# vbronetskyi/nclt-slam-project

Measured on AMD Instinct MI355X. Metric: relocalization frames/sec @640x480, 10k-landmark DB; Hamming-match HBM GB/s, higher is better.
Workload: dtype u8; 1 GPU; 640x480 BGR frames, 10000-record landmark DB (640000 descriptors, rows=fixed64), global relocalization tick per frame: ORB(500) + whole-DB mutual Hamming scan + top-25 PnP-RANSAC(200); frames resident in HBM, every frame's 96-byte result record written to pinned host memory by the tick's last kernel; distinct_frames=32, preroll_steps=20, streams=4, records=10000, descriptors=640000, parallelism=frames sharded across ranks, database replicated, no collective

## Files before the change

nclt-slam-project_amd/csrc/reloc_ctx.hip:

```cpp
#include <stdarg.h>
#include <stdlib.h>

#include "reloc_internal.h"

static thread_local char g_err[512] = "";

void reloc_set_error(const char *fmt, ...)
{
    va_list ap;
    va_start(ap, fmt);
    vsnprintf(g_err, sizeof(g_err), fmt, ap);
    va_end(ap);
}

RELOC_API const char *reloc_last_error(void) { return g_err; }

RELOC_API int reloc_device_count(void)
{
    int n = 0;
    if (hipGetDeviceCount(&n) != hipSuccess) return 0;
    return n;
}

template <typename T>
// ... 68 lines not shown
    int n = 0;
    if (hipGetDeviceCount(&n) != hipSuccess || n <= 0) {
        reloc_set_error("no HIP device available (libreloc_hip has no CPU fallback)");
        return nullptr;
    }
    if (device < 0 || device >= n || max_w < 64 || max_h < 64 || max_feat < 64) {
        reloc_set_error("reloc_create: bad arguments (device %d of %d, %dx%d, max_feat %d)", device, n,
                        max_w, max_h, max_feat);
        return nullptr;
    }
    if (hipSetDevice(device) != hipSuccess) {
        reloc_set_error("hipSetDevice(%d) failed", device);
        return nullptr;
    }
    reloc_ctx *c = new reloc_ctx();
    __atomic_add_fetch(&g_reloc_live_contexts, 1, __ATOMIC_RELAXED);
    c->device = device;
    c->max_w = max_w;
    c->max_h = max_h;
    c->max_feat = max_feat;
    hipDeviceProp_t prop;
    if (hipGetDeviceProperties(&prop, device) == hipSuccess) c->num_cu = prop.multiProcessorCount;
    if (hipStreamCreateWithFlags(&c->own_stream, hipStreamNonBlocking) != hipSuccess ||
        hipEventCreate(&c->t0) != hipSuccess || hipEventCreate(&c->t1) != hipSuccess) {
        reloc_set_error("stream/event creation failed");
        __atomic_sub_fetch(&g_reloc_live_contexts, 1, __ATOMIC_RELAXED);
        delete c;
        return nullptr;
    }
    c->stream = c->own_stream;
    c->prm.nfeatures = 500;
    c->prm.max_candidates = RELOC_MAX_CANDIDATES;
    c->prm.min_matches = RELOC_MIN_MATCHES;
    c->prm.min_inliers = RELOC_MIN_INLIERS;
    c->prm.ransac_iterations = RELOC_RANSAC_ITERATIONS;
    c->prm.global_max_candidates = RELOC_GLOBAL_MAX_CANDIDATES;
    c->prm.global_min_inliers = RELOC_GLOBAL_MIN_INLIERS;
    c->prm.accum_min_kpts = RELOC_ACCUM_MIN_KPTS;
    c->prm.candidate_radius_m = RELOC_CANDIDATE_RADIUS_M;
    c->prm.heading_tol_deg = RELOC_HEADING_TOL_DEG;
    c->prm.reproj_max_px = RELOC_REPROJ_MAX_PX;
    c->prm.ransac_reproj_px = RELOC_RANSAC_REPROJ_PX;
    c->prm.ransac_confidence = RELOC_RANSAC_CONFIDENCE;
    c->prm.consistency_m = RELOC_CONSISTENCY_M;
    c->prm.global_reproj_max_px = RELOC_GLOBAL_REPROJ_MAX_PX;
    c->prm.accum_min_dist_m = RELOC_ACCUM_MIN_DIST_M;
    c->prm.accum_depth_min_m = RELOC_ACCUM_DEPTH_MIN_M;
    c->prm.accum_depth_max_m = RELOC_ACCUM_DEPTH_MAX_M;
    c->prm.gray_coeff_bits = RELOC_GRAY_DEFAULT_BITS;
    c->prm.reserved0 = 0;
    if (const char *dev = getenv("RELOC_DEV"); dev && dev[0] == '1' && dev[1] == 0) {
        if (const char *e = getenv("RELOC_SCAN_GRID")) c->scan_grid = atoi(e);
        if (const char *e = getenv("RELOC_SCAN_GENS")) c->scan_gens = atoi(e);
        if (const char *e = getenv("RELOC_SCAN_NW")) c->scan_nw = atoi(e);
        if (const char *e = getenv("RELOC_SCAN_BATCH_GENS")) c->scan_batch_gens = atoi(e);
        if (const char *e = getenv("RELOC_SCAN_QUOTA_ROWS")) c->scan_quota_rows = atoi(e);
        if (const char *e = getenv("RELOC_LOCAL_TWO_STAGE")) c->local_two_stage = atoi(e) != 0;
    }
    if (ctx_alloc(c) != 0) {
        reloc_destroy(c);
        return nullptr;
    }
    return c;
}

RELOC_API void reloc_destroy(reloc_ctx *c)
{
    if (!c) return;
    (void)hipSetDevice(c->device);
    if (c->stream) (void)hipStreamSynchronize(c->stream);
    db_arrays_drop(c->db_share, c->db_desc, c->db_pts3d, c->db_kp2d, c->db_off, c->db_pose, c->db_xy_heading);
    void *ptrs[] = {c->pyr, c->blur, c->nms, c->rz_tab, c->pyr_tiles, c->hist, c->cand_cnt, c->cand_key, c->cand_resp,
                    c->kp_cnt, c->kp_key, c->kp_resp, c->f_xy, c->f_size, c->f_angle, c->f_resp, c->f_oct,
                    c->f_desc, c->f_count, c->frame_img, c->orb_const, c->dbg_cut, c->db_counts, c->topk_part, c->cand_ids, c->cand_n, c->m_qidx,
                    c->m_tidx, c->m_dist, c->m_n, c->p_obj, c->p_img, c->p_Rt, c->p_cnt, c->p_inl,
                    c->p_out, c->tick_res, c->accum_res, c->tick_flags, c->scan_ticket, c->clahe_plane, c->clahe_lut};
    for (void *p : ptrs)
        if (p) (void)hipFree(p);
    if (c->tick_res_host) (void)hipHostFree(c->tick_res_host);
    {
        DbArena &a = c->db_slot[1 - c->db_sel];
        db_arrays_drop(a.share, a.desc, a.pts3d, a.kp2d, a.off, a.pose, a.xy_heading);
        if (a.counts) (void)hipFree(a.counts);
        if (a.topk_part) (void)hipFree(a.topk_part);
    }
    for (int i = 0; i < 8; ++i)
        if (c->scratch[i]) (void)hipFree(c->scratch[i]);
    for (int k = 0; k < RELOC_PROF_N; ++k)
        if (c->prof[k].init)
            for (int i = 0; i < RELOC_PROF_RING; ++i) {
                (void)hipEventDestroy(c->prof[k].a[i]);
                (void)hipEventDestroy(c->prof[k].b[i]);
            }
    if (c->t0) (void)hipEventDestroy(c->t0);
    if (c->t1) (void)hipEventDestroy(c->t1);
    if (c->own_stream) (void)hipStreamDestroy(c->own_stream);
    __atomic_sub_fetch(&g_reloc_live_contexts, 1, __ATOMIC_RELAXED);
    delete c;
}

RELOC_API int reloc_get_params(reloc_ctx *c, reloc_params *out)
{
    ARG_CHECK_CTX(c, out, "reloc_get_params");
    *out = c->prm;
    return RELOC_OK;
}

// ... 184 lines not shown
```

nclt-slam-project_amd/csrc/reloc_internal.h:

```cpp
#pragma once
#include <hip/hip_runtime.h>
#include <stdint.h>
#include <stdio.h>
#include <string.h>

#include "../../include/reloc.h"
#include "../../include/reloc_spec.h"

#define RELOC_API extern "C" __attribute__((visibility("default")))
#define RELOC_PROF_RING 256

void reloc_set_error(const char *fmt, ...);

#define HIP_TRY(expr)                                                                      \
    do {                                                                                   \
        hipError_t e_ = (expr);                                                            \
        if (e_ != hipSuccess) {                                                            \
            reloc_set_error("%s failed: %s (%s:%d)", #expr, hipGetErrorString(e_), __FILE__, \
                            __LINE__);                                                     \
            return RELOC_E_HIP;                                                            \
        }                                                                                  \
    } while (0)

#define ARG_CHECK(cond, msg)                                 \
// ... 205 lines not shown
    int max_w = 0, max_h = 0, max_feat = 0;
    hipStream_t own_stream = nullptr;
    hipStream_t stream = nullptr;
    hipEvent_t t0 = nullptr, t1 = nullptr;
    int num_cu = 256;

    int prof_on = 0;
    struct ProfSlot { hipEvent_t a[RELOC_PROF_RING], b[RELOC_PROF_RING]; int n = 0; float total = 0.f; int launches = 0; bool init = false; } prof[RELOC_PROF_N];

    void *scratch[8] = {};
    int64_t scratch_bytes[8] = {};

    int orb_w = 0, orb_h = 0, orb_nfeat = 0;
    OrbLevel lev[NLEV];
    int64_t pyr_bytes = 0;
    uint8_t *pyr = nullptr;
    uint8_t *blur = nullptr;
    uint8_t *nms = nullptr;
    int32_t *rz_tab = nullptr;
    void *pyr_tiles = nullptr;
    int pyr_ntiles = 0, pyr_lds[NLEV + 1] = {}, pyr_lds_bytes = 0;
    int32_t *hist = nullptr;
    int32_t *cand_cnt = nullptr;
    uint32_t *cand_key = nullptr;
    float *cand_resp = nullptr;
    int32_t *kp_cnt = nullptr;
    uint32_t *kp_key = nullptr;
    float *kp_resp = nullptr;
    float *f_xy = nullptr, *f_size = nullptr, *f_angle = nullptr, *f_resp = nullptr;
    int32_t *f_oct = nullptr;
    uint8_t *f_desc = nullptr;
    int32_t *f_count = nullptr;
    uint8_t *frame_img = nullptr;
    void *orb_const = nullptr;
    char orb_tab_host[1024];
    int32_t *dbg_cut = nullptr;

    double K4[4] = {RELOC_FX, RELOC_FY, RELOC_CX, RELOC_CY};
    double b2c_t[3] = {0.35, 0.0, 0.18};
    double b2c_R[9] = {0, -1, 0, 0, 0, -1, 1, 0, 0};
    double dist[5] = {0, 0, 0, 0, 0};
    bool has_dist = false;

    double clahe_clip = 0.0;
    int clahe_tx = 0, clahe_ty = 0;
    uint8_t *clahe_plane = nullptr;
    uint8_t *clahe_lut = nullptr;

    reloc_params prm;
    int scan_grid = 0;
    int scan_gens = 0;
    int scan_batch_gens = 0;
    int scan_quota_rows = 1;
    int scan_nw = 0;
    uint32_t *scan_ticket = nullptr;

    DbArena db_slot[2];
    int db_sel = 0;
    bool db_shared = false;
    DbShare *db_share = nullptr;
    int64_t db_records = 0, db_rows = 0;
    int64_t db_cap_records = 0, db_cap_rows = 0;
    int db_max_rows = 0;
    uint8_t *db_desc = nullptr;
    float *db_pts3d = nullptr;
    float *db_kp2d = nullptr;
    int64_t *db_off = nullptr;
    double *db_pose = nullptr;
    double *db_xy_heading = nullptr;
    int32_t *db_counts = nullptr;
    unsigned long long *topk_part = nullptr;
    int topk_blocks = 0;
    AccumResult *accum_res = nullptr;
    int32_t *tick_flags = nullptr;

    int32_t *cand_ids = nullptr;
    int32_t *cand_n = nullptr;
    int32_t *m_qidx = nullptr, *m_tidx = nullptr, *m_dist = nullptr, *m_n = nullptr;
    float *p_obj = nullptr, *p_img = nullptr;
    double *p_Rt = nullptr;
    int32_t *p_cnt = nullptr;
    int32_t *p_inl = nullptr;
    PnpOut *p_out = nullptr;
    int exclusive_hint = -1;
    bool orb_latency_shape = true;
    bool latency_shapes = false;
    bool local_two_stage = false;
    TickResult *tick_res = nullptr;
    TickResult *tick_res_host = nullptr;
    bool tick_failed = false;
    int32_t tick_seq = 0;
    TickResult *tick_res_ext = nullptr;
};

int reloc_scratch(reloc_ctx *ctx, int slot, int64_t bytes, void **out);
void reloc_prof_begin(reloc_ctx *ctx, int which);
void reloc_prof_end(reloc_ctx *ctx, int which);

void db_arrays_drop(DbShare *&share, uint8_t *&desc, float *&pts3d, float *&kp2d, int64_t *&off, double *&pose, double *&xyh);
extern int g_reloc_live_contexts;
static inline bool ctx_alone(const reloc_ctx *c)
{
    return c->exclusive_hint > 0 || (c->exclusive_hint < 0 && __atomic_load_n(&g_reloc_live_contexts, __ATOMIC_RELAXED) == 1);
}

int launch_db_scan(reloc_ctx *ctx, const uint8_t *db_desc, const int64_t *db_off, int64_t n_rec,
                   const int32_t *rec_ids, const int32_t *n_ids_dev, int n_ids_max, const uint8_t *cur,
// ... 17 lines not shown
```

nclt-slam-project_amd/csrc/reloc_match.hip:

```cpp
#include <stdlib.h>
#include <new>
#include <type_traits>
#include <utility>

#include "reloc_internal.h"

typedef uint32_t u32;

__device__ __forceinline__ u32 bcnt_acc(u32 x, u32 acc)
{
    u32 r;
    asm("v_bcnt_u32_b32 %0, %1, %2" : "=v"(r) : "v"(x), "v"(acc));
    return r;
}
__device__ __forceinline__ u32 min_u16(u32 a, u32 b)
{
    u32 r;
    asm("v_min_u16 %0, %1, %2" : "=v"(r) : "v"(a), "v"(b));
    return r;
}
template <u32 IDX>
__device__ __forceinline__ u32 key_fma(u32 d, u32 c128)
{
    u32 r;
// ... 275 lines not shown
                for (; tc < tend; tc += 16)
                    scan_chunk<NJ, 16, true>(rec, n, tc, min(16, tend - tc), q, (u32)(cb * CB), rowkey, colbest, ncb == 1, lane);
            }
        }
        __syncthreads();
        u32 base = 0;
        for (int rb = 0; rb < n; rb += 64 * NW) {
            const int row = rb + tid;
            bool mutual = false;
            u32 key = 0;
            if (row < n && C > 0) {
                key = rowkey[row];
                const u32 col = key & 0xFFFFu;
                mutual = (colbest[col] & 0xFFFFu) == (u32)row;
            }
            const unsigned long long bal = __ballot(mutual);
            if (lane == 0) wsum[wave] = (u32)__popcll(bal);
            __syncthreads();
            u32 before = base;
            for (int w = 0; w < wave; ++w) before += wsum[w];
            u32 total = 0;
            for (int w = 0; w < NW; ++w) total += wsum[w];
            if (EMIT && mutual) {
                const u32 pos = before + (u32)__popcll(bal & ((1ull << lane) - 1ull));
                const int64_t o = (int64_t)it * emit_stride + pos;
                m_qidx[o] = row;
                m_tidx[o] = (int32_t)(key & 0xFFFFu);
                m_dist[o] = (int32_t)(key >> 16);
                if (mask.g_obj) {
                    const float *p3 = mask.g_pts3d + 3 * (row0 + row), *p2 = mask.g_xy + 2 * (size_t)(key & 0xFFFFu);
                    float *po = mask.g_obj + 3 * o, *pi = mask.g_img + 2 * o;
                    po[0] = p3[0]; po[1] = p3[1]; po[2] = p3[2];
                    pi[0] = p2[0]; pi[1] = p2[1];
                }
            }
            base += total;
            __syncthreads();
        }
        if (tid == 0) {
            if (counts) counts[EMIT ? it : r] = (int32_t)base;
            if (EMIT && m_n) m_n[it] = (int32_t)base;
        }
        advance();
    }
    if (ticket && tid == 0) {
        const int words = pool_frames * 8;
        if (atomicAdd(&ticket_pool[words * TICKET_STRIDE], 1u) == gridDim.x - 1) {
            for (int x = 0; x <= words; ++x)
                __hip_atomic_store(&ticket_pool[x * TICKET_STRIDE], 0u, __ATOMIC_RELAXED, __HIP_MEMORY_SCOPE_AGENT);
        }
    }
}

template <int NJ, int NW>
__device__ __forceinline__ void db_count_body(
    u32 *lds, int C, const uint4 *__restrict__ db, const int64_t *__restrict__ off, const int32_t *__restrict__ rec_ids,
    const int32_t *__restrict__ n_ids_p, int n_ids_max, const uint4 *__restrict__ cur, int max_rows,
    int32_t *__restrict__ counts, const ScanMask &mask, u32 *ticket, int quota, int n_bounded, int col_words,
    u32 *ticket_pool = nullptr, int pool_frames = 1, int block = -1, int n_blocks = -1)
{
    if (!ticket_pool) ticket_pool = ticket;
    if (block < 0) { block = blockIdx.x; n_blocks = gridDim.x; }
    constexpr int CB = 64 * NJ;
    const int tid = threadIdx.x, lane = tid & 63;
    const int wave = __builtin_amdgcn_readfirstlane(tid >> 6);
    const int n_ids = n_ids_p ? min(*n_ids_p, n_ids_max) : n_ids_max;
    const int ncb = max((C + CB - 1) / CB, 1);
    const bool dbl = 2 * ncb * CB <= col_words;
    u32 *colbuf = lds;
    u32 *rowkey = colbuf + col_words;
    u32 *wsum = rowkey + max_rows;

    u32 q[NJ][8];
    auto load_q = [&](int colbase) {
#pragma unroll
        for (int j = 0; j < NJ; ++j) {
            const int col = min(colbase + j * 64 + lane, max(C - 1, 0));
            const uint4 a = cur[2 * col], b = cur[2 * col + 1];
            q[j][0] = a.x; q[j][1] = a.y; q[j][2] = a.z; q[j][3] = a.w;
            q[j][4] = b.x; q[j][5] = b.y; q[j][6] = b.z; q[j][7] = b.w;
        }
    };
    const bool bound = (NW % ncb) == 0;
    const int my_cb = bound ? wave % ncb : 0;
    const int chunk0 = bound ? wave / ncb : wave, chunk_step = bound ? NW / ncb : NW;
    const bool stand_down = mask.skip_if && *mask.skip_if != 0;
    if (bound && !stand_down) load_q(my_cb * CB);
    double hc = 1.0, hs = 0.0, cos_tol = 0.0;
    if (mask.xyh) {
        cur_heading_q(mask.q, hc, hs);
        cos_tol = mask.cos_tol;
        hc = uniform_f64(hc); hs = uniform_f64(hs); cos_tol = uniform_f64(cos_tol);
    }
    constexpr int TICKET_STRIDE = 32;
    int shard = 0, dry = 0;
    if (ticket) {
        u32 x;
        asm volatile("s_getreg_b32 %0, hwreg(HW_REG_XCC_ID, 0, 4)" : "=s"(x));
        shard = (int)(x & 7u);
    }
    auto draw = [&]() -> u32 { return atomicAdd(&ticket[shard * TICKET_STRIDE], 1u); };
    auto settle = [&](u32 t) -> int {
        for (;;) {
            const long long rec_i = (long long)n_blocks + (long long)shard + 8ll * (long long)t;
            if (rec_i < n_ids) return (int)rec_i;
            if (++dry >= 8) return n_ids;
            shard = (shard + 1) & 7;
            t = draw();
        }
    };
    int it = stand_down ? n_ids : block;
    const bool by_rows = n_bounded >= 0;
    int left = (quota > 0 && (!by_rows || block < n_bounded)) ? quota : 0x7fffffff;
    for (int i = tid; i < ncb * CB; i += 64 * NW) colbuf[i] = 0xFFFFFFFFu;
    if (tid == 0) wsum[0] = wsum[1] = 0;
    __syncthreads();
    int p = 0;
    while (it < n_ids) {
        u32 *colbest = colbuf + (dbl ? p * ncb * CB : 0);
        const int r = rec_ids ? rec_ids[it] : it;
        const bool scored = !(mask.xyh && !heading_ok(mask.xyh + 4 * (int64_t)r, hc, hs, cos_tol));
        const int64_t row0 = off[r];
        const int n = scored ? (int)(off[r + 1] - row0) : 0;
        const uint4 *rec = db + 2 * row0;
        left -= by_rows ? max(n, 1) : 1;
        u32 next_ticket = 0;
        if (ticket && tid == 0 && left > 0) next_ticket = draw();
        if (n > 0 && C > 0) {
            if (ncb > 1) {
                for (int i = tid; i < n; i += 64 * NW) rowkey[i] = 0xFFFFFFFFu;
                __syncthreads();
            }
            for (int cb = bound ? my_cb : 0; cb < (bound ? my_cb + 1 : ncb); ++cb) {
                if (!bound) load_q(cb * CB);
                const int per = n / chunk_step, extra = n % chunk_step;
                int tc = chunk0 * per + min(chunk0, extra);
                const int tend = tc + per + (chunk0 < extra ? 1 : 0);
#pragma nounroll
                for (; tc < tend; tc += 16)
                    scan_chunk<NJ, 16, true>(rec, n, tc, min(16, tend - tc), q, (u32)(cb * CB), rowkey, colbest, ncb == 1, lane);
            }
        }
        if (dbl) {
            u32 *other = colbuf + (p ^ 1) * ncb * CB;
            for (int i = tid; i < ncb * CB; i += 64 * NW) other[i] = 0xFFFFFFFFu;
        }
        __syncthreads();
        if (C > 0) {
            for (int rb = 0; rb < n; rb += 64 * NW) {
                const int row = rb + tid;
                bool mutual = false;
                if (row < n) {
                    const u32 col = rowkey[row] & 0xFFFFu;
                    mutual = (colbest[col] & 0xFFFFu) == (u32)row;
                }
                const u32 c = (u32)__popcll(__ballot(mutual));
                if (lane == 0 && c) atomicAdd(&wsum[p], c);
            }
        }
        if (tid == 0) wsum[8] = ticket ? (left > 0 ? (u32)settle(next_ticket) : (u32)n_ids) : (u32)(it + n_blocks);
        __syncthreads();
        if (tid == 0) {
            counts[r] = (int32_t)wsum[p];
            wsum[p] = 0;
        }
        it = __builtin_amdgcn_readfirstlane((int)wsum[8]);
        if (dbl) p ^= 1;
        else {
            for (int i = tid; i < ncb * CB; i += 64 * NW) colbuf[i] = 0xFFFFFFFFu;
            __syncthreads();
        }
    }
    if (ticket && tid == 0) {
        const int words = pool_frames * 8;
        if (atomicAdd(&ticket_pool[words * TICKET_STRIDE], 1u) == gridDim.x - 1) {
            for (int x = 0; x <= words; ++x)
                __hip_atomic_store(&ticket_pool[x * TICKET_STRIDE], 0u, __ATOMIC_RELAXED, __HIP_MEMORY_SCOPE_AGENT);
        }
    }
}

template <int NJ, bool EMIT, int NW>
__global__ __launch_bounds__(64 * NW, NW >= 4 ? 16 / NW : 4) RELOC_SCAN_VGPR_ATTR void k_db_scan(
    const uint4 *__restrict__ db, const int64_t *__restrict__ off, const int32_t *__restrict__ rec_ids,
    const int32_t *__restrict__ n_ids_p, int n_ids_max, const uint4 *__restrict__ cur,
    const int32_t *__restrict__ n_cur_p, int n_cur_max, int max_rows, int32_t *__restrict__ counts,
    int32_t *__restrict__ m_qidx, int32_t *__restrict__ m_tidx, int32_t *__restrict__ m_dist,
    int32_t *__restrict__ m_n, int emit_stride, ScanMask mask, u32 *ticket, int quota, int n_bounded, int col_words)
{
    extern __shared__ u32 lds[];
    if constexpr (EMIT) RELOC_SMALL_KERNEL_PRIO();
    const int C = n_cur_p ? min(*n_cur_p, n_cur_max) : n_cur_max;
    if constexpr (EMIT)
        db_scan_body<NJ, true, NW>(lds, C, db, off, rec_ids, n_ids_p, n_ids_max, cur, max_rows, counts, m_qidx, m_tidx, m_dist, m_n,
                                   emit_stride, mask, ticket, quota);
    else
        db_count_body<NJ, NW>(lds, C, db, off, rec_ids, n_ids_p, n_ids_max, cur, max_rows, counts, mask, ticket, quota, n_bounded, col_words);
}

struct EmitFrame {
    const int32_t *rec_ids, *n_ids_p; const uint4 *cur; const int32_t *n_cur_p;
    int32_t *m_qidx, *m_tidx, *m_dist, *m_n; const float *g_xy; float *g_obj, *g_img;
};
struct EmitBatch { EmitFrame f[RELOC_BATCH_MAX]; };

__global__ __launch_bounds__(256, 4) RELOC_SCAN_VGPR_ATTR void k_db_emit_batch(const uint4 *__restrict__ db, const int64_t *__restrict__ off, int n_ids_max,
                                                          int n_cur_max, int max_rows, int emit_stride, const float *__restrict__ g_pts3d,
                                                          EmitBatch bt)
{
    extern __shared__ u32 lds[];
    RELOC_SMALL_KERNEL_PRIO();
    const EmitFrame &F = bt.f[blockIdx.y];
    ScanMask mask;
    mask.xyh = nullptr;
    mask.q[0] = mask.q[1] = mask.q[2] = 0; mask.q[3] = 1;
    mask.g_pts3d = g_pts3d; mask.g_xy = F.g_xy; mask.g_obj = F.g_obj; mask.g_img = F.g_img;
    const int C = F.n_cur_p ? min(*F.n_cur_p, n_cur_max) : n_cur_max;
    db_scan_body<8, true, 4>(lds, C, db, off, F.rec_ids, F.n_ids_p, n_ids_max, F.cur, max_rows, nullptr, F.m_qidx, F.m_tidx, F.m_dist, F.m_n,
                             emit_stride, mask, nullptr, 0);
}

int launch_db_emit_batch(reloc_ctx *const *ctxs, int n)
{
    reloc_ctx *c0 = ctxs[0];
    if (n < 1 || n > RELOC_BATCH_MAX) { reloc_set_error("emit batch: 1..%d frames", RELOC_BATCH_MAX); return RELOC_E_ARG; }
    if (c0->max_feat > 65535 || c0->db_max_rows > MAX_REC_ROWS) { reloc_set_error("emit batch: capacity"); return RELOC_E_CAPACITY; }
    EmitBatch bt;
    for (int f = 0; f < RELOC_BATCH_MAX; ++f) {
        reloc_ctx *c = ctxs[f < n ? f : 0];
        EmitFrame &F = bt.f[f];
        F.rec_ids = c->cand_ids; F.n_ids_p = c->cand_n; F.cur = (const uint4 *)c->f_desc; F.n_cur_p = c->f_count;
        F.m_qidx = c->m_qidx; F.m_tidx = c->m_tidx; F.m_dist = c->m_dist; F.m_n = c->m_n; F.g_xy = c->f_xy; F.g_obj = c->p_obj; F.g_img = c->p_img;
    }
    const int max_rows = c0->db_max_rows < 1 ? 1 : c0->db_max_rows;
    const int ncb = (c0->max_feat + 511) / 512;
    const size_t lds = (size_t)(ncb * 512 + max_rows + 16) * 4;
    if (lds > 160 * 1024) { reloc_set_error("emit batch: LDS demand %zu bytes", lds); return RELOC_E_CAPACITY; }
    hipLaunchKernelGGL(k_db_emit_batch, dim3(MAX_CAND, n), dim3(256), lds, c0->stream, (const uint4 *)c0->db_desc, c0->db_off, MAX_CAND,
                       c0->max_feat, max_rows, MAX_REC_ROWS, c0->db_pts3d, bt);
    HIP_TRY(hipGetLastError());
    return RELOC_OK;
}

constexpr int SCAN_BATCH_MAX = 8;
struct ScanBatch {
    int n;
    const uint4 *cur[SCAN_BATCH_MAX];
    const int32_t *n_cur[SCAN_BATCH_MAX];
    int32_t *counts[SCAN_BATCH_MAX];
    const int32_t *skip_if[SCAN_BATCH_MAX];
    double q[SCAN_BATCH_MAX][4];
    const double *xyh;
    double cos_tol;
};

__global__ __launch_bounds__(256, 4) RELOC_SCAN_VGPR_ATTR void k_db_scan_batch(const uint4 *__restrict__ db, const int64_t *__restrict__ off, int n_ids,
                                                          int n_cur_max, int max_rows, ScanBatch bt, u32 *ticket_pool, int quota, int n_bounded, int col_words)
{
    extern __shared__ u32 lds[];
    const int f = blockIdx.x % bt.n;
    ScanMask mask;
    mask.xyh = bt.xyh;
    for (int k = 0; k < 4; ++k) mask.q[k] = bt.q[f][k];
    mask.cos_tol = bt.cos_tol;
    mask.skip_if = bt.skip_if[f];
    const int C = bt.n_cur[f] ? min(*bt.n_cur[f], n_cur_max) : n_cur_max;
    db_count_body<8, 4>(lds, C, db, off, nullptr, nullptr, n_ids, bt.cur[f], max_rows, bt.counts[f], mask, ticket_pool + f * 8 * 32, quota,
                        n_bounded, col_words, ticket_pool, bt.n, (int)(blockIdx.x / bt.n), (int)((gridDim.x + bt.n - 1 - f) / bt.n));
}

__device__ __forceinline__ u32 max_u16(u32 a, u32 b)
{
    u32 r;
    asm("v_max_u16 %0, %1, %2" : "=v"(r) : "v"(a), "v"(b));
    return r;
}

__global__ __launch_bounds__(256, 4) void k_db_ratio(const uint4 *__restrict__ db, const int64_t *__restrict__ off, int n_rec,
                                                     const uint4 *__restrict__ cur, const int32_t *__restrict__ n_cur_p,
                                                     int n_cur_max, double ratio, int32_t *__restrict__ counts)
{
    __shared__ u32 s_part[4][512];
    __shared__ int s_cnt[4];
    const int tid = threadIdx.x, lane = tid & 63;
    const int wave = __builtin_amdgcn_readfirstlane(tid >> 6);
    const int C = n_cur_p ? min(*n_cur_p, n_cur_max) : n_cur_max;
    const int ncb = max((C + 511) >> 9, 1);
    u32 q[8][8];
    auto load_q = [&](int colbase) {
#pragma unroll
        for (int j = 0; j < 8; ++j) {
            const int col = min(colbase + j * 64 + lane, max(C - 1, 0));
            const uint4 a = cur[2 * col], b = cur[2 * col + 1];
            q[j][0] = a.x; q[j][1] = a.y; q[j][2] = a.z; q[j][3] = a.w;
            q[j][4] = b.x; q[j][5] = b.y; q[j][6] = b.z; q[j][7] = b.w;
        }
    };
    if (ncb == 1 && C > 0) load_q(0);
    for (int r = blockIdx.x; r < n_rec; r += gridDim.x) {
        const int64_t row0 = off[r];
        const int n = (int)(off[r + 1] - row0);
        const uint4 *rec = db + 2 * row0;
        int good = 0;
        if (n >= 2 && C > 0) {
            for (int cb = 0; cb < ncb; ++cb) {
                if (ncb > 1) load_q(cb * 512);
                u32 k0[8], k1[8];
#pragma unroll
                for (int j = 0; j < 8; ++j) { k0[j] = 0xFFFFu; k1[j] = 0xFFFFu; }
                for (int t0 = wave * 8; t0 < n; t0 += 32) {
                    auto row_of = [&](int t) { return min(t0 + t, n - 1); };
                    uint4 a = rec[2 * row_of(0)], b = rec[2 * row_of(0) + 1];
#pragma unroll
                    for (int t = 0; t < 8; ++t) {
                        srow_landed(a.x);
                        uint4 na, nb;
                        if (t + 1 < 8) { na = rec[2 * row_of(t + 1)]; nb = rec[2 * row_of(t + 1) + 1]; }
                        __builtin_amdgcn_sched_barrier(0);
                        if (t0 + t < n) {
#pragma unroll
                            for (int j = 0; j < 8; j += 2) {
// ... 211 lines not shown
            if (n <= 64) {
                const u32 peer = (u32)__builtin_amdgcn_ds_bpermute((int)(sq_lane_of<G>(rb & 63u) << 2), (int)colk);
                total = __popcll(__ballot(lane < n && (peer & 0xFFFFu) == (u32)lane));
                if (lane == 0) counts[r] = total;
                continue;
            }
            rowk[lane] = (unsigned short)rb;
        }
        for (int tc = 64; tc < n; tc += 64) {
            const int row = min(tc + lane, n - 1);
            const u32 rb = chunk(rec[2 * row], rec[2 * row + 1], tc, colk);
            if (tc + lane < n) rowk[tc + lane] = (unsigned short)rb;
        }
        total = 0;
        for (int tc = 0; tc < n; tc += 64) {
            const u32 k = tc + lane < n ? rowk[tc + lane] : 0u;
            const u32 peer = (u32)__builtin_amdgcn_ds_bpermute((int)(sq_lane_of<G>(k & 63u) << 2), (int)colk);
            total += __popcll(__ballot(tc + lane < n && (peer & 0xFFFFu) == (u32)(tc + lane)));
        }
        if (lane == 0) counts[r] = total;
    }
}

int launch_db_scan(reloc_ctx *ctx, const uint8_t *db_desc, const int64_t *db_off, int64_t n_rec,
                   const int32_t *rec_ids, const int32_t *n_ids_dev, int n_ids_max, const uint8_t *cur,
                   const int32_t *n_cur_dev, int n_cur_max, int max_rows, int32_t *counts, int32_t *m_qidx,
                   int32_t *m_tidx, int32_t *m_dist, int32_t *m_n, int emit_stride, const ScanMask *mask_p)
{
    if (n_ids_max <= 0) return RELOC_OK;
    ScanMask mask;
    mask.xyh = nullptr;
    mask.q[0] = mask.q[1] = mask.q[2] = 0; mask.q[3] = 1;
    if (mask_p) mask = *mask_p;
    if (n_cur_max > 65535) { reloc_set_error("db scan: more than 65535 current descriptors"); return RELOC_E_CAPACITY; }
    if (max_rows > MAX_REC_ROWS) { reloc_set_error("db scan: record larger than %d rows", MAX_REC_ROWS); return RELOC_E_CAPACITY; }
    if (max_rows < 1) max_rows = 1;
    if (!m_qidx && !rec_ids && !n_ids_dev && !mask.xyh && counts && n_cur_max <= 64 && max_rows <= SQ_MAX_ROWS) {
        if (n_cur_max == 0) {
            HIP_TRY(hipMemsetAsync(counts, 0, (size_t)n_ids_max * sizeof(int32_t), ctx->stream));
            return RELOC_OK;
        }
        int grid = ctx->num_cu * 8;
        const int need = (n_ids_max + SQ_WAVES - 1) / SQ_WAVES;
        if (grid > need) grid = need;
#define RELOC_LAUNCH_ROWS(G, HOIST)                                                                                           \
    hipLaunchKernelGGL((k_db_scan_rows<G, HOIST>), dim3(grid), dim3(64 * SQ_WAVES), 0, ctx->stream, (const uint4 *)db_desc, db_off, n_ids_max, \
                       (const uint4 *)cur, n_cur_dev, n_cur_max, counts)
        if (n_cur_max <= 4) RELOC_LAUNCH_ROWS(4, true); else if (n_cur_max <= 8) RELOC_LAUNCH_ROWS(8, false); else RELOC_LAUNCH_ROWS(16, false);
#undef RELOC_LAUNCH_ROWS
        HIP_TRY(hipGetLastError());
        return RELOC_OK;
    }
    const int nj = n_cur_max <= 128 ? 2 : (n_cur_max <= 256 ? 4 : 8);
    const int cb = 64 * nj;
    const int ncb = (n_cur_max + cb - 1) / cb > 0 ? (n_cur_max + cb - 1) / cb : 1;
    const int col_words = (m_qidx || ncb >= 2 ? ncb : 2) * cb;
    const size_t lds = (size_t)(col_words + max_rows + 16) * 4;
    if (lds > 160 * 1024) { reloc_set_error("db scan: LDS demand %zu bytes", lds); return RELOC_E_CAPACITY; }
    int nw = 4;
    if (!m_qidx && nj == 8) {
        nw = ctx->scan_nw == 1 || ctx->scan_nw == 2 || ctx->scan_nw == 4 ? ctx->scan_nw : 4;
        if (nw == 1 && lds * 16 > 150 * 1024) nw = 2;
    }
    int wg_per_cu = 16 / nw;
    if ((size_t)wg_per_cu * lds > 160 * 1024) wg_per_cu = (int)(160 * 1024 / lds);
    const int resident = ctx->num_cu * wg_per_cu;
    int grid = ctx->scan_grid > 0 ? ctx->scan_grid : ctx->num_cu * 16;
    u32 *ticket = nullptr;
    int quota = 0, n_bounded = 0;
    if (!rec_ids && !n_ids_dev && n_ids_max > resident && ctx->scan_ticket && ctx->scan_grid >= 0 && nj == 8) {
        ticket = ctx->scan_ticket;
        const int gens = ctx->scan_gens > 0 ? ctx->scan_gens : (RELOC_SCAN_GENS_SHARED > 0 ? RELOC_SCAN_GENS_SHARED : 1);
        const int q_rec = (n_ids_max + resident * gens - 1) / (resident * gens);
        n_bounded = (n_ids_max + q_rec - 1) / q_rec;
        grid = n_bounded + 8 < n_ids_max ? n_bounded + 8 : n_ids_max;
        const int64_t rows = db_desc == ctx->db_desc && ctx->db_rows > 0 ? ctx->db_rows : (int64_t)n_ids_max * 64;
        quota = (int)((rows * q_rec + n_ids_max - 1) / n_ids_max);
        if (quota < 1) quota = 1;
        if (!ctx->scan_quota_rows) { quota = q_rec; grid = n_bounded; n_bounded = -1; }
        if ((ctx_alone(ctx) || RELOC_SCAN_GENS_SHARED == 0) && ctx->scan_gens == 0) { quota = 0; grid = resident; }
        if (ctx->scan_gens < 0) { quota = 0; grid = ctx->scan_gens <= -2 ? ctx->num_cu * (-ctx->scan_gens - 1) : resident; }
    }
    if (grid > n_ids_max) grid = n_ids_max;
#define RELOC_LAUNCH_SCAN(NJ, EMIT, NW)                                                                                      \
    hipLaunchKernelGGL((k_db_scan<NJ, EMIT, NW>), dim3(grid), dim3(64 * NW), lds, ctx->stream, (const uint4 *)db_desc, db_off, rec_ids, \
                       n_ids_dev, n_ids_max, (const uint4 *)cur, n_cur_dev, n_cur_max, max_rows, counts, m_qidx, m_tidx, m_dist, \
                       m_n, emit_stride, mask, ticket, quota, n_bounded, col_words)
    if (m_qidx && ctx->latency_shapes) {
        if (nj == 2) RELOC_LAUNCH_SCAN(2, true, 8); else if (nj == 4) RELOC_LAUNCH_SCAN(4, true, 8); else RELOC_LAUNCH_SCAN(8, true, 8);
    } else if (m_qidx) {
        if (nj == 2) RELOC_LAUNCH_SCAN(2, true, 4); else if (nj == 4) RELOC_LAUNCH_SCAN(4, true, 4); else RELOC_LAUNCH_SCAN(8, true, 4);
    } else if (nj == 8) {
        if (nw == 1) RELOC_LAUNCH_SCAN(8, false, 1); else if (nw == 2) RELOC_LAUNCH_SCAN(8, false, 2); else RELOC_LAUNCH_SCAN(8, false, 4);
    } else {
        if (nj == 2) RELOC_LAUNCH_SCAN(2, false, 4); else RELOC_LAUNCH_SCAN(4, false, 4);
    }
#undef RELOC_LAUNCH_SCAN
    HIP_TRY(hipGetLastError());
    return RELOC_OK;
}

int launch_db_scan_batch(reloc_ctx *const *ctxs, int n, const double *q, double cos_tol, bool auto_mode, bool heading_mask)
{
    reloc_ctx *c0 = ctxs[0];
    if (n < 1 || n > SCAN_BATCH_MAX) { reloc_set_error("scan batch: 1..%d frames", SCAN_BATCH_MAX); return RELOC_E_ARG; }
    if (c0->max_feat > 65535 || c0->db_max_rows > MAX_REC_ROWS) { reloc_set_error("scan batch: capacity"); return RELOC_E_CAPACITY; }
    ScanBatch bt;
    bt.n = n;
    bt.xyh = heading_mask ? c0->db_xy_heading : nullptr;
    bt.cos_tol = cos_tol;
    for (int f = 0; f < SCAN_BATCH_MAX; ++f) {
        reloc_ctx *c = ctxs[f < n ? f : 0];
        bt.cur[f] = (const uint4 *)c->f_desc; bt.n_cur[f] = c->f_count; bt.counts[f] = c->db_counts;
        bt.skip_if[f] = auto_mode ? c->cand_n : nullptr;
        for (int k = 0; k < 4; ++k) bt.q[f][k] = q[4 * (f < n ? f : 0) + k];
    }
    const int n_ids = (int)c0->db_records, max_rows = c0->db_max_rows < 1 ? 1 : c0->db_max_rows;
    const int ncb = (c0->max_feat + 511) / 512;
    const int col_words = (ncb >= 2 ? ncb : 2) * 512;
    const size_t lds_all = (size_t)(col_words + max_rows + 16) * 4;
    int gens = c0->scan_gens > 0 ? c0->scan_gens : (RELOC_SCAN_GENS_SHARED > 0 ? RELOC_SCAN_GENS_SHARED : 1);
    if (c0->scan_batch_gens > 0) gens = c0->scan_batch_gens;
    const int resident = c0->num_cu * 4;
    int per_frame = (resident * gens + n - 1) / n;
    if (per_frame > n_ids) per_frame = n_ids;
    if (per_frame < 1) per_frame = 1;
    const int q_rec = (n_ids + per_frame - 1) / per_frame;
    const int n_bounded = (n_ids + q_rec - 1) / q_rec;
    int quota = (int)(((c0->db_rows > 0 ? c0->db_rows : (int64_t)n_ids * 64) * q_rec + n_ids - 1) / n_ids);
    if (quota < 1) quota = 1;
    per_frame = n_bounded + 1;
    if (per_frame > n_ids) per_frame = n_ids;
    int nb_arg = n_bounded;
    if (!c0->scan_quota_rows) { quota = q_rec; per_frame = n_bounded; nb_arg = -1; }
    hipLaunchKernelGGL(k_db_scan_batch, dim3(per_frame * n), dim3(256), lds_all, c0->stream, (const uint4 *)c0->db_desc, c0->db_off,
                       n_ids, c0->max_feat, max_rows, bt, c0->scan_ticket, quota, nb_arg, col_words);
    HIP_TRY(hipGetLastError());
    return RELOC_OK;
}

__global__ __launch_bounds__(256) void k_knn2(const uint4 *__restrict__ A, int na, const uint4 *__restrict__ B,
                                              int nb, int rows_per_split, u32 *__restrict__ part)
{
    const int i = blockIdx.x * 256 + threadIdx.x;
    const int j0 = blockIdx.y * rows_per_split;
    const int j1 = min(nb, j0 + rows_per_split);
    u32 q[8] = {0, 0, 0, 0, 0, 0, 0, 0};
    if (i < na) {
        const uint4 a = A[2 * i], b = A[2 * i + 1];
        q[0] = a.x; q[1] = a.y; q[2] = a.z; q[3] = a.w;
        q[4] = b.x; q[5] = b.y; q[6] = b.z; q[7] = b.w;
    }
    u32 k0 = 0xFFFFFFFFu, k1 = 0xFFFFFFFFu;
#pragma unroll 4
    for (int j = j0; j < j1; ++j) {
        const u32 h = ham8(q, B[2 * j], B[2 * j + 1], 0);
        const u32 key = (h << 22) | (u32)j;
        const u32 m = umax(k0, key);
        k0 = umin(k0, key);
        k1 = umin(k1, m);
    }
    if (i < na) {
        part[((size_t)blockIdx.y * na + i) * 2] = k0;
        part[((size_t)blockIdx.y * na + i) * 2 + 1] = k1;
    }
}

__global__ void k_knn2_merge(const u32 *__restrict__ part, int na, int nsplit, int32_t *__restrict__ idx,
                             int32_t *__restrict__ dist)
{
    const int i = blockIdx.x * blockDim.x + threadIdx.x;
    if (i >= na) return;
    u32 k0 = 0xFFFFFFFFu, k1 = 0xFFFFFFFFu;
    for (int s = 0; s < nsplit; ++s)
        for (int e = 0; e < 2; ++e) {
            const u32 key = part[((size_t)s * na + i) * 2 + e];
            const u32 m = umax(k0, key);
            k0 = umin(k0, key);
            k1 = umin(k1, m);
        }
    idx[2 * i] = k0 == 0xFFFFFFFFu ? -1 : (int32_t)(k0 & 0x3FFFFFu);
    dist[2 * i] = k0 == 0xFFFFFFFFu ? -1 : (int32_t)(k0 >> 22);
    idx[2 * i + 1] = k1 == 0xFFFFFFFFu ? -1 : (int32_t)(k1 & 0x3FFFFFu);
    dist[2 * i + 1] = k1 == 0xFFFFFFFFu ? -1 : (int32_t)(k1 >> 22);
}

constexpr int MAT_ROWS = 128;
constexpr int MAT_UNIT_ROWS = 8;
// ... 582 lines not shown
```

Baseline: 7305 frames/s.

## Compute Hamming mutual-match counting scan with int8 MFMA matrix ops

Replaces the popcount-based counting DB scan with an MFMA kernel. Each 256-bit descriptor is split into nibble bit-planes encoded as int8 so that a 32x32x32 i8 MFMA produces packed Hamming distances, with popcount and row-index bias terms folded into an extra K slice. Row and column minima are then reduced with DPP and permlane swaps and combined through LDS atomics. The aim is to move the XOR-popcount ALU work onto matrix cores with 8-wave workgroups. The cost is a more intricate encoding, more LDS use and fewer workgroups per CU, and the old NW tuning knob is removed.

```diff
diff --git a/nclt-slam-project_amd/csrc/reloc_ctx.hip b/nclt-slam-project_amd/csrc/reloc_ctx.hip
--- a/nclt-slam-project_amd/csrc/reloc_ctx.hip
+++ b/nclt-slam-project_amd/csrc/reloc_ctx.hip
@@ -144,7 +144,6 @@
     if (const char *dev = getenv("RELOC_DEV"); dev && dev[0] == '1' && dev[1] == 0) {
         if (const char *e = getenv("RELOC_SCAN_GRID")) c->scan_grid = atoi(e);
         if (const char *e = getenv("RELOC_SCAN_GENS")) c->scan_gens = atoi(e);
-        if (const char *e = getenv("RELOC_SCAN_NW")) c->scan_nw = atoi(e);
         if (const char *e = getenv("RELOC_SCAN_BATCH_GENS")) c->scan_batch_gens = atoi(e);
         if (const char *e = getenv("RELOC_SCAN_QUOTA_ROWS")) c->scan_quota_rows = atoi(e);
         if (const char *e = getenv("RELOC_LOCAL_TWO_STAGE")) c->local_two_stage = atoi(e) != 0;
diff --git a/nclt-slam-project_amd/csrc/reloc_internal.h b/nclt-slam-project_amd/csrc/reloc_internal.h
--- a/nclt-slam-project_amd/csrc/reloc_internal.h
+++ b/nclt-slam-project_amd/csrc/reloc_internal.h
@@ -281,7 +281,6 @@
     int scan_gens = 0;
     int scan_batch_gens = 0;
     int scan_quota_rows = 1;
-    int scan_nw = 0;
     uint32_t *scan_ticket = nullptr;
 
     DbArena db_slot[2];
diff --git a/nclt-slam-project_amd/csrc/reloc_match.hip b/nclt-slam-project_amd/csrc/reloc_match.hip
--- a/nclt-slam-project_amd/csrc/reloc_match.hip
+++ b/nclt-slam-project_amd/csrc/reloc_match.hip
@@ -351,8 +351,23 @@
     }
 }
 
-template <int NJ, int NW>
-__device__ __forceinline__ void db_count_body(
+constexpr int MF_WAVES = 8;
+constexpr int MF_CB = 512;
+constexpr int MF_WG_PER_CU = 2;
+constexpr int MF_GROUP = 64;
+constexpr int MF_AIMG_WORDS = (MF_GROUP / 32) * 9 * 64 * 4;
+typedef int v4i_t __attribute__((ext_vector_type(4)));
+typedef int v16i_t __attribute__((ext_vector_type(16)));
+
+__device__ __forceinline__ u32 mf_byte(int v) { return (u32)v & 0xFFu; }
+__device__ __forceinline__ void mf_settle(v16i_t &p0, v16i_t &p1)
+{
+    asm volatile("s_nop 7\n\ts_nop 7\n\ts_nop 7" : "+v"(p0), "+v"(p1));
+}
+
+__host__ __device__ constexpr size_t mf_lds_words(int col_words, int max_rows) { return (size_t)MF_AIMG_WORDS + col_words + max_rows + 16; }
+
+__device__ __forceinline__ void db_count_mfma_body(
     u32 *lds, int C, const uint4 *__restrict__ db, const int64_t *__restrict__ off, const int32_t *__restrict__ rec_ids,
     const int32_t *__restrict__ n_ids_p, int n_ids_max, const uint4 *__restrict__ cur, int max_rows,
     int32_t *__restrict__ counts, const ScanMask &mask, u32 *ticket, int quota, int n_bounded, int col_words,
@@ -360,31 +375,43 @@
 {
     if (!ticket_pool) ticket_pool = ticket;
     if (block < 0) { block = blockIdx.x; n_blocks = gridDim.x; }
-    constexpr int CB = 64 * NJ;
+    constexpr int NT = MF_WAVES * 64;
     const int tid = threadIdx.x, lane = tid & 63;
     const int wave = __builtin_amdgcn_readfirstlane(tid >> 6);
+    const int c = lane & 31, h = lane >> 5;
     const int n_ids = n_ids_p ? min(*n_ids_p, n_ids_max) : n_ids_max;
-    const int ncb = max((C + CB - 1) / CB, 1);
-    const bool dbl = 2 * ncb * CB <= col_words;
-    u32 *colbuf = lds;
-    u32 *rowkey = colbuf + col_words;
+    const int ncb = max((C + MF_CB - 1) / MF_CB, 1);
+    v4i_t *aimg = reinterpret_cast<v4i_t *>(lds);
+    u32 *colbest = lds + MF_AIMG_WORDS;
+    u32 *rowkey = colbest + col_words;
     u32 *wsum = rowkey + max_rows;
 
-    u32 q[NJ][8];
-    auto load_q = [&](int colbase) {
-#pragma unroll
-        for (int j = 0; j < NJ; ++j) {
-            const int col = min(colbase + j * 64 + lane, max(C - 1, 0));
-            const uint4 a = cur[2 * col], b = cur[2 * col + 1];
-            q[j][0] = a.x; q[j][1] = a.y; q[j][2] = a.z; q[j][3] = a.w;
-            q[j][4] = b.x; q[j][5] = b.y; q[j][6] = b.z; q[j][7] = b.w;
+    v4i_t B[2][9];
+    auto load_b = [&](int cb) {
+#pragma unroll
+        for (int t = 0; t < 2; ++t) {
+            const int col = min(cb * MF_CB + 32 * (2 * wave + t) + c, max(C - 1, 0));
+            const uint4 lo = cur[2 * col], hi = cur[2 * col + 1];
+            const u32 w[8] = {lo.x, lo.y, lo.z, lo.w, hi.x, hi.y, hi.z, hi.w};
+            int pc = 0;
+#pragma unroll
+            for (int s = 0; s < 8; ++s) {
+                const u32 x = w[s] >> (4 * h);
+                B[t][s] = v4i_t{(int)((x << 1) & 0x02020202u), (int)(x & 0x02020202u), (int)((x >> 1) & 0x02020202u),
+                                (int)((x >> 2) & 0x02020202u)};
+                pc += __popc(w[s]);
+            }
+            const int q0 = min(pc, 128), q1 = pc - q0;
+            B[t][8] = v4i_t{0, 0, 0, 0};
+            if (h == 0) {
+                B[t][8].x = (int)(0x8080u | (mf_byte(-q0) << 16) | (mf_byte(-q1) << 24));
+                B[t][8].y = (int)(1u | ((u32)t << 8) | (0x80u << 16) | (0x80u << 24));
+                B[t][8].z = (int)0x80u;
+            }
         }
     };
-    const bool bound = (NW % ncb) == 0;
-    const int my_cb = bound ? wave % ncb : 0;
-    const int chunk0 = bound ? wave / ncb : wave, chunk_step = bound ? NW / ncb : NW;
     const bool stand_down = mask.skip_if && *mask.skip_if != 0;
-    if (bound && !stand_down) load_q(my_cb * CB);
+    if (ncb == 1 && C > 0 && !stand_down) load_b(0);
     double hc = 1.0, hs = 0.0, cos_tol = 0.0;
     if (mask.xyh) {
         cur_heading_q(mask.q, hc, hs);
@@ -411,12 +438,10 @@
     int it = stand_down ? n_ids : block;
     const bool by_rows = n_bounded >= 0;
     int left = (quota > 0 && (!by_rows || block < n_bounded)) ? quota : 0x7fffffff;
-    for (int i = tid; i < ncb * CB; i += 64 * NW) colbuf[i] = 0xFFFFFFFFu;
-    if (tid == 0) wsum[0] = wsum[1] = 0;
-    __syncthreads();
-    int p = 0;
+    if (tid == 0) wsum[0] = 0;
+    const int bg = ((lane >> 1) & 1) + 2 * ((lane >> 4) & 1) + 4 * ((lane >> 3) & 1) + 8 * ((lane >> 2) & 1);
+    const int brow = (bg & 3) + 8 * (bg >> 2) + 4 * h;
     while (it < n_ids) {
-        u32 *colbest = colbuf + (dbl ? p * ncb * CB : 0);
         const int r = rec_ids ? rec_ids[it] : it;
         const bool scored = !(mask.xyh && !heading_ok(mask.xyh + 4 * (int64_t)r, hc, hs, cos_tol));
         const int64_t row0 = off[r];
@@ -426,49 +451,123 @@
         u32 next_ticket = 0;
         if (ticket && tid == 0 && left > 0) next_ticket = draw();
         if (n > 0 && C > 0) {
-            if (ncb > 1) {
-                for (int i = tid; i < n; i += 64 * NW) rowkey[i] = 0xFFFFFFFFu;
+            for (int i = tid; i < ncb * MF_CB; i += NT) colbest[i] = 0xFFFFFFFFu;
+            for (int i = tid; i < n; i += NT) rowkey[i] = 0xFFFFFFFFu;
+            for (int g0 = 0; g0 < n; g0 += MF_GROUP) {
+                if (g0 > 0) __syncthreads();
+                {
+                    const int rt = (tid >> 6) & 1, sq = tid >> 7;
+                    const int row = g0 + 32 * rt + c;
+                    const bool real = row < n;
+                    const uint4 *rp = rec + 2 * (real ? row : 0);
+                    const uint4 lo = rp[0], hi = rp[1];
+                    const u32 w[8] = {lo.x, lo.y, lo.z, lo.w, hi.x, hi.y, hi.z, hi.w};
+#pragma unroll
+                    for (int k = 0; k < 2; ++k) {
+                        const int s = 2 * sq + k;
+                        u32 ws = w[0];
+#pragma unroll
+                        for (int j = 1; j < 8; ++j) ws = s == j ? w[j] : ws;
+                        const u32 x = real ? ws >> (4 * h) : 0u;
+                        aimg[(rt * 9 + s) * 64 + lane] = v4i_t{(int)((x << 7) & 0x80808080u), (int)((x << 6) & 0x80808080u),
+                                                               (int)((x << 5) & 0x80808080u), (int)((x << 4) & 0x80808080u)};
+                    }
+                    if (sq == 0) {
+                        v4i_t a8 = v4i_t{0, 0, 0, 0};
+                        if (h == 0) {
+                            const u32 rowpart = 8u * (u32)((c & 3) + 4 * (c >> 3));
+                            if (real) {
+                                int pc = 0;
+#pragma unroll
+                                for (int j = 0; j < 8; ++j) pc += __popc(w[j]);
+                                const int p0 = min(pc, 128), p1 = pc - p0;
+                                a8.x = (int)(mf_byte(-p0) | (mf_byte(-p1) << 8) | (0x80u << 16) | (0x80u << 24));
+                                a8.y = (int)(rowpart | (1u << 8));
+                            } else {
+                                a8.y = (int)(rowpart | (1u << 8) | (0x80u << 16) | (0x80u << 24));
+                                a8.z = (int)0xFFu;
+                            }
+                        }
+                        aimg[(rt * 9 + 8) * 64 + lane] = a8;
+                    }
+                }
                 __syncthreads();
+                const int ntile = min(n - g0, MF_GROUP) > 32 ? 2 : 1;
+                for (int cb = 0; cb < ncb; ++cb) {
+                    if (ncb > 1) load_b(cb);
+                    const u32 colbase = (u32)(cb * MF_CB + 64 * wave);
+                    u32 cbk0 = 0xFFFFFFFFu, cbk1 = 0xFFFFFFFFu;
+                    for (int rt = 0; rt < ntile; ++rt) {
+                        v16i_t P0 = v16i_t{0, 0, 0, 0, 0, 0, 0, 0, 0, 0, 0, 0, 0, 0, 0, 0}, P1 = P0;
+#pragma unroll
+                        for (int s = 0; s < 9; ++s) {
+                            const v4i_t a = aimg[(rt * 9 + s) * 64 + lane];
+                            P0 = __builtin_amdgcn_mfma_i32_32x32x32_i8(a, B[0][s], P0, 0, 0, 0);
+                            P1 = __builtin_amdgcn_mfma_i32_32x32x32_i8(a, B[1][s], P1, 0, 0, 0);
+                        }
+                        mf_settle(P0, P1);
+                        u32 m0 = (u32)P0[0], m1 = (u32)P1[0];
+                        u32 x[16];
+#pragma unroll
+                        for (int g = 0; g < 16; ++g) {
+                            if (g) { m0 = min_u16(m0, (u32)P0[g]); m1 = min_u16(m1, (u32)P1[g]); }
+                            x[g] = min_u16((u32)P0[g], (u32)P1[g]);
+                        }
+                        const u32 rtile = (u32)(g0 + 32 * rt + 4 * h);
+                        {
+                            const u32 g_0 = (m0 >> 3) & 15u, g_1 = (m1 >> 3) & 15u;
+                            cbk0 = umin(cbk0, ((m0 >> 7) << 16) | (rtile + (g_0 & 3u) + 8u * (g_0 >> 2)));
+                            cbk1 = umin(cbk1, ((m1 >> 7) << 16) | (rtile + (g_1 & 3u) + 8u * (g_1 >> 2)));
+                        }
+#pragma unroll
+                        for (int g = 0; g < 16; ++g) x[g] = (x[g] << 5) | (u32)c;
+#pragma unroll
+                        for (int g = 0; g < 8; ++g) x[g] = bfly_dpp<4>(x[g], x[g + 8]);
+#pragma unroll
+                        for (int g = 0; g < 4; ++g) x[g] = bfly_dpp<8>(x[g], x[g + 4]);
+#pragma unroll
+                        for (int g = 0; g < 2; ++g) x[g] = bfly<16>(x[g], x[g + 2], lane);
+                        u32 v = bfly<2>(x[0], x[1], lane);
+                        asm("s_nop 1\n\tv_min_u32_dpp %0, %0, %0 quad_perm:[1,0,3,2] row_mask:0xf bank_mask:0xf" : "+v"(v));
+                        const int row = g0 + 32 * rt + brow;
+                        if ((lane & 1) == 0 && row < n) {
+                            const u32 col = colbase + 32u * ((v >> 5) & 7u) + (v & 31u);
+                            atomicMin(&rowkey[row], ((v >> 12) << 16) | col);
+                        }
+                    }
+                    {
+                        const auto s0 = __builtin_amdgcn_permlane32_swap(cbk0, cbk0, false, false);
+                        const auto s1 = __builtin_amdgcn_permlane32_swap(cbk1, cbk1, false, false);
+                        cbk0 = umin(s0[0], s0[1]);
+                        cbk1 = umin(s1[0], s1[1]);
+                    }
+                    if (h == 0) {
+                        atomicMin(&colbest[colbase + c], cbk0);
+                        atomicMin(&colbest[colbase + 32 + c], cbk1);
+                    }
+                }
             }
-            for (int cb = bound ? my_cb : 0; cb < (bound ? my_cb + 1 : ncb); ++cb) {
-                if (!bound) load_q(cb * CB);
-                const int per = n / chunk_step, extra = n % chunk_step;
-                int tc = chunk0 * per + min(chunk0, extra);
-                const int tend = tc + per + (chunk0 < extra ? 1 : 0);
-#pragma nounroll
-                for (; tc < tend; tc += 16)
-                    scan_chunk<NJ, 16, true>(rec, n, tc, min(16, tend - tc), q, (u32)(cb * CB), rowkey, colbest, ncb == 1, lane);
-            }
-        }
-        if (dbl) {
-            u32 *other = colbuf + (p ^ 1) * ncb * CB;
-            for (int i = tid; i < ncb * CB; i += 64 * NW) other[i] = 0xFFFFFFFFu;
         }
         __syncthreads();
         if (C > 0) {
-            for (int rb = 0; rb < n; rb += 64 * NW) {
+            for (int rb = 0; rb < n; rb += NT) {
                 const int row = rb + tid;
                 bool mutual = false;
                 if (row < n) {
                     const u32 col = rowkey[row] & 0xFFFFu;
                     mutual = (colbest[col] & 0xFFFFu) == (u32)row;
                 }
-                const u32 c = (u32)__popcll(__ballot(mutual));
-                if (lane == 0 && c) atomicAdd(&wsum[p], c);
+                const u32 cnt = (u32)__popcll(__ballot(mutual));
+                if (lane == 0 && cnt) atomicAdd(&wsum[0], cnt);
             }
         }
         if (tid == 0) wsum[8] = ticket ? (left > 0 ? (u32)settle(next_ticket) : (u32)n_ids) : (u32)(it + n_blocks);
         __syncthreads();
         if (tid == 0) {
-            counts[r] = (int32_t)wsum[p];
-            wsum[p] = 0;
+            counts[r] = (int32_t)wsum[0];
+            wsum[0] = 0;
         }
         it = __builtin_amdgcn_readfirstlane((int)wsum[8]);
-        if (dbl) p ^= 1;
-        else {
-            for (int i = tid; i < ncb * CB; i += 64 * NW) colbuf[i] = 0xFFFFFFFFu;
-            __syncthreads();
-        }
     }
     if (ticket && tid == 0) {
         const int words = pool_frames * 8;
@@ -485,16 +584,25 @@
     const int32_t *__restrict__ n_ids_p, int n_ids_max, const uint4 *__restrict__ cur,
     const int32_t *__restrict__ n_cur_p, int n_cur_max, int max_rows, int32_t *__restrict__ counts,
     int32_t *__restrict__ m_qidx, int32_t *__restrict__ m_tidx, int32_t *__restrict__ m_dist,
-    int32_t *__restrict__ m_n, int emit_stride, ScanMask mask, u32 *ticket, int quota, int n_bounded, int col_words)
-{
+    int32_t *__restrict__ m_n, int emit_stride, ScanMask mask, u32 *ticket, int quota)
+{
+    static_assert(EMIT, "the counting scan is k_db_scan_mfma");
     extern __shared__ u32 lds[];
-    if constexpr (EMIT) RELOC_SMALL_KERNEL_PRIO();
+    RELOC_SMALL_KERNEL_PRIO();
     const int C = n_cur_p ? min(*n_cur_p, n_cur_max) : n_cur_max;
-    if constexpr (EMIT)
-        db_scan_body<NJ, true, NW>(lds, C, db, off, rec_ids, n_ids_p, n_ids_max, cur, max_rows, counts, m_qidx, m_tidx, m_dist, m_n,
-                                   emit_stride, mask, ticket, quota);
-    else
-        db_count_body<NJ, NW>(lds, C, db, off, rec_ids, n_ids_p, n_ids_max, cur, max_rows, counts, mask, ticket, quota, n_bounded, col_words);
+    db_scan_body<NJ, true, NW>(lds, C, db, off, rec_ids, n_ids_p, n_ids_max, cur, max_rows, counts, m_qidx, m_tidx, m_dist, m_n,
+                               emit_stride, mask, ticket, quota);
+}
+
+__global__ __launch_bounds__(64 * MF_WAVES, MF_WG_PER_CU * MF_WAVES / 4) void k_db_scan_mfma(
+    const uint4 *__restrict__ db, const int64_t *__restrict__ off, const int32_t *__restrict__ rec_ids,
+    const int32_t *__restrict__ n_ids_p, int n_ids_max, const uint4 *__restrict__ cur,
+    const int32_t *__restrict__ n_cur_p, int n_cur_max, int max_rows, int32_t *__restrict__ counts,
+    ScanMask mask, u32 *ticket, int quota, int n_bounded, int col_words)
+{
+    extern __shared__ u32 lds[];
+    const int C = n_cur_p ? min(*n_cur_p, n_cur_max) : n_cur_max;
+    db_count_mfma_body(lds, C, db, off, rec_ids, n_ids_p, n_ids_max, cur, max_rows, counts, mask, ticket, quota, n_bounded, col_words);
 }
 
 struct EmitFrame {
@@ -553,7 +661,7 @@
     double cos_tol;
 };
 
-__global__ __launch_bounds__(256, 4) RELOC_SCAN_VGPR_ATTR void k_db_scan_batch(const uint4 *__restrict__ db, const int64_t *__restrict__ off, int n_ids,
+__global__ __launch_bounds__(64 * MF_WAVES, MF_WG_PER_CU * MF_WAVES / 4) void k_db_scan_batch(const uint4 *__restrict__ db, const int64_t *__restrict__ off, int n_ids,
                                                           int n_cur_max, int max_rows, ScanBatch bt, u32 *ticket_pool, int quota, int n_bounded, int col_words)
 {
     extern __shared__ u32 lds[];
@@ -564,8 +672,8 @@
     mask.cos_tol = bt.cos_tol;
     mask.skip_if = bt.skip_if[f];
     const int C = bt.n_cur[f] ? min(*bt.n_cur[f], n_cur_max) : n_cur_max;
-    db_count_body<8, 4>(lds, C, db, off, nullptr, nullptr, n_ids, bt.cur[f], max_rows, bt.counts[f], mask, ticket_pool + f * 8 * 32, quota,
-                        n_bounded, col_words, ticket_pool, bt.n, (int)(blockIdx.x / bt.n), (int)((gridDim.x + bt.n - 1 - f) / bt.n));
+    db_count_mfma_body(lds, C, db, off, nullptr, nullptr, n_ids, bt.cur[f], max_rows, bt.counts[f], mask, ticket_pool + f * 8 * 32, quota,
+                       n_bounded, col_words, ticket_pool, bt.n, (int)(blockIdx.x / bt.n), (int)((gridDim.x + bt.n - 1 - f) / bt.n));
 }
 
 __device__ __forceinline__ u32 max_u16(u32 a, u32 b)
@@ -883,23 +991,19 @@
         return RELOC_OK;
     }
     const int nj = n_cur_max <= 128 ? 2 : (n_cur_max <= 256 ? 4 : 8);
-    const int cb = 64 * nj;
+    const int cb = m_qidx ? 64 * nj : MF_CB;
     const int ncb = (n_cur_max + cb - 1) / cb > 0 ? (n_cur_max + cb - 1) / cb : 1;
-    const int col_words = (m_qidx || ncb >= 2 ? ncb : 2) * cb;
-    const size_t lds = (size_t)(col_words + max_rows + 16) * 4;
+    const int col_words = ncb * cb;
+    const size_t lds = m_qidx ? (size_t)(col_words + max_rows + 16) * 4 : mf_lds_words(col_words, max_rows) * 4;
     if (lds > 160 * 1024) { reloc_set_error("db scan: LDS demand %zu bytes", lds); return RELOC_E_CAPACITY; }
-    int nw = 4;
-    if (!m_qidx && nj == 8) {
-        nw = ctx->scan_nw == 1 || ctx->scan_nw == 2 || ctx->scan_nw == 4 ? ctx->scan_nw : 4;
-        if (nw == 1 && lds * 16 > 150 * 1024) nw = 2;
-    }
-    int wg_per_cu = 16 / nw;
+    const int nw = m_qidx ? 4 : MF_WAVES;
+    int wg_per_cu = m_qidx ? 16 / nw : MF_WG_PER_CU;
     if ((size_t)wg_per_cu * lds > 160 * 1024) wg_per_cu = (int)(160 * 1024 / lds);
     const int resident = ctx->num_cu * wg_per_cu;
     int grid = ctx->scan_grid > 0 ? ctx->scan_grid : ctx->num_cu * 16;
     u32 *ticket = nullptr;
     int quota = 0, n_bounded = 0;
-    if (!rec_ids && !n_ids_dev && n_ids_max > resident && ctx->scan_ticket && ctx->scan_grid >= 0 && nj == 8) {
+    if (!rec_ids && !n_ids_dev && n_ids_max > resident && ctx->scan_ticket && ctx->scan_grid >= 0 && (!m_qidx || nj == 8)) {
         ticket = ctx->scan_ticket;
         const int gens = ctx->scan_gens > 0 ? ctx->scan_gens : (RELOC_SCAN_GENS_SHARED > 0 ? RELOC_SCAN_GENS_SHARED : 1);
         const int q_rec = (n_ids_max + resident * gens - 1) / (resident * gens);
@@ -916,15 +1020,15 @@
 #define RELOC_LAUNCH_SCAN(NJ, EMIT, NW)                                                                                      \
     hipLaunchKernelGGL((k_db_scan<NJ, EMIT, NW>), dim3(grid), dim3(64 * NW), lds, ctx->stream, (const uint4 *)db_desc, db_off, rec_ids, \
                        n_ids_dev, n_ids_max, (const uint4 *)cur, n_cur_dev, n_cur_max, max_rows, counts, m_qidx, m_tidx, m_dist, \
-                       m_n, emit_stride, mask, ticket, quota, n_bounded, col_words)
+                       m_n, emit_stride, mask, ticket, quota)
     if (m_qidx && ctx->latency_shapes) {
         if (nj == 2) RELOC_LAUNCH_SCAN(2, true, 8); else if (nj == 4) RELOC_LAUNCH_SCAN(4, true, 8); else RELOC_LAUNCH_SCAN(8, true, 8);
     } else if (m_qidx) {
         if (nj == 2) RELOC_LAUNCH_SCAN(2, true, 4); else if (nj == 4) RELOC_LAUNCH_SCAN(4, true, 4); else RELOC_LAUNCH_SCAN(8, true, 4);
-    } else if (nj == 8) {
-        if (nw == 1) RELOC_LAUNCH_SCAN(8, false, 1); else if (nw == 2) RELOC_LAUNCH_SCAN(8, false, 2); else RELOC_LAUNCH_SCAN(8, false, 4);
     } else {
-        if (nj == 2) RELOC_LAUNCH_SCAN(2, false, 4); else RELOC_LAUNCH_SCAN(4, false, 4);
+        hipLaunchKernelGGL(k_db_scan_mfma, dim3(grid), dim3(64 * MF_WAVES), lds, ctx->stream, (const uint4 *)db_desc, db_off, rec_ids,
+                           n_ids_dev, n_ids_max, (const uint4 *)cur, n_cur_dev, n_cur_max, max_rows, counts, mask, ticket, quota, n_bounded,
+                           col_words);
     }
 #undef RELOC_LAUNCH_SCAN
     HIP_TRY(hipGetLastError());
@@ -947,12 +1051,12 @@
         for (int k = 0; k < 4; ++k) bt.q[f][k] = q[4 * (f < n ? f : 0) + k];
     }
     const int n_ids = (int)c0->db_records, max_rows = c0->db_max_rows < 1 ? 1 : c0->db_max_rows;
-    const int ncb = (c0->max_feat + 511) / 512;
-    const int col_words = (ncb >= 2 ? ncb : 2) * 512;
-    const size_t lds_all = (size_t)(col_words + max_rows + 16) * 4;
+    const int col_words = (c0->max_feat + MF_CB - 1) / MF_CB * MF_CB > 0 ? (c0->max_feat + MF_CB - 1) / MF_CB * MF_CB : MF_CB;
+    const size_t lds_all = mf_lds_words(col_words, max_rows) * 4;
+    if (lds_all > 160 * 1024) { reloc_set_error("scan batch: LDS demand %zu bytes", lds_all); return RELOC_E_CAPACITY; }
     int gens = c0->scan_gens > 0 ? c0->scan_gens : (RELOC_SCAN_GENS_SHARED > 0 ? RELOC_SCAN_GENS_SHARED : 1);
     if (c0->scan_batch_gens > 0) gens = c0->scan_batch_gens;
-    const int resident = c0->num_cu * 4;
+    const int resident = c0->num_cu * MF_WG_PER_CU;
     int per_frame = (resident * gens + n - 1) / n;
     if (per_frame > n_ids) per_frame = n_ids;
     if (per_frame < 1) per_frame = 1;
@@ -964,7 +1068,7 @@
     if (per_frame > n_ids) per_frame = n_ids;
     int nb_arg = n_bounded;
     if (!c0->scan_quota_rows) { quota = q_rec; per_frame = n_bounded; nb_arg = -1; }
-    hipLaunchKernelGGL(k_db_scan_batch, dim3(per_frame * n), dim3(256), lds_all, c0->stream, (const uint4 *)c0->db_desc, c0->db_off,
+    hipLaunchKernelGGL(k_db_scan_batch, dim3(per_frame * n), dim3(64 * MF_WAVES), lds_all, c0->stream, (const uint4 *)c0->db_desc, c0->db_off,
                        n_ids, c0->max_feat, max_rows, bt, c0->scan_ticket, quota, nb_arg, col_words);
     HIP_TRY(hipGetLastError());
     return RELOC_OK;
```

New measurement: 7989 frames/s, median of 6. 1.09x the previous value.
